# davrempe/contact-human-dynamics

Hardware: NVIDIA H100
Metric: optimised frames/sec (batched phys-optim) (higher is better)
Workload: dtype f64

## Files before the change

### contact-human-dynamics_b200/csrc/chd_api.cu

```cuda
#include <cuda_runtime.h>

#include <cstdio>
#include <cstdlib>
#include <cstring>
#include <vector>

#include "../../include/chd.h"
#include "chd_dev.h"

__global__ void chd_k_stage_begin(ChdDev D);
template <bool GLOBAL>
__global__ void chd_k_eval(ChdDev D);
__global__ void chd_k_init(ChdDev D);
__global__ void chd_k_kkt(ChdDev D);
__global__ void chd_k_kkt_gwin(ChdDev D);
__global__ void chd_k_kcopy(ChdDev D);
__global__ void chd_k_curv(ChdDev D);
__global__ void chd_k_asm(ChdDev D);
__global__ void chd_k_fp64_peak(int mode, int iters, double* sink);
__global__ void chd_k_hess_base(ChdDev D);
__global__ void chd_k_hess_dur(ChdDev D);
__global__ void chd_k_hess_zero(ChdDev D);
__global__ void chd_k_hess_fin(ChdDev D, int mode);
__global__ void chd_k_tables(ChdDev D);
// ... 31 lines not shown
struct chd_phys_batch {
  ChdHostBatch hb;
  ChdDev D;
  std::vector<void*> allocs;
  cudaStream_t stream = nullptr, copy_stream = nullptr;
  cudaEvent_t ev_kkt = nullptr, ev_ls = nullptr, ev_copy = nullptr;
  int64_t launches = 0;
  int timing = 0;
  bool host_only = false;
  double kt_ms[KT_N] = {0};
  int64_t kt_n[KT_N] = {0};
  cudaEvent_t ev0 = nullptr, ev1 = nullptr;
  int* d_frames = nullptr;
  double* d_samples = nullptr;
  ChdIterForm iter = {};
  size_t smem_kkt = 0;
  int kcopy_blocks = 1;
  ChdIpm* h_ipm = nullptr;
  double* d_x0 = nullptr;
  int64_t h2d_bytes = 0;
  ChdStageDev* d_stages = nullptr;
  int sched_max_iter = 0;
  bool sched_has_dur = false;
  double *poly_T0 = nullptr, *poly_tend0 = nullptr, *phase_tend0 = nullptr;
  int* ent_col0 = nullptr;
};

namespace {

template <class T>
// ... 38 lines not shown
    b->launches++;
    b->kt_n[id]++;
    if (b->timing) {
      cudaEventRecord(b->ev1, b->stream);
      cudaEventSynchronize(b->ev1);
      float ms = 0;
      cudaEventElapsedTime(&ms, b->ev0, b->ev1);
      b->kt_ms[id] += ms;
    }
  }
};

void launch_eval(chd_phys_batch* b) {
  Timer t(b, KT_EVAL);
  b->iter.eval<<<b->hb.B, CHD_THREADS, b->iter.smem_eval, b->stream>>>(b->D);
}

int set_schedule(chd_phys_batch* b, const int* sched, int nsched, int override_stage, int override_max_iter) {
  ChdStageDev tab[6];
  for (int s = 0; s < 6; ++s) tab[s] = stage_dev(b->hb.stage[s], s);
  if (override_stage >= 0 && override_max_iter > 0) tab[override_stage].max_iter = override_max_iter;
  CHD_CUDA(cudaMemcpyAsync(b->d_stages, tab, sizeof(tab), cudaMemcpyHostToDevice, b->stream));
  b->D.stages = b->d_stages;
  b->D.nsched = nsched;
  for (int i = 0; i < nsched; ++i) b->D.sched[i] = sched[i];
  b->sched_max_iter = 0;
  b->sched_has_dur = false;
  for (int i = 0; i < nsched; ++i) b->sched_max_iter += tab[sched[i]].max_iter + 2, b->sched_has_dur |= sched[i] == CHD_STAGE_3;
  chd_k_sched_reset<<<(b->hb.B + 127) / 128, 128, 0, b->stream>>>(b->D);
  b->launches++;
  return 0;
}

int run_schedule(chd_phys_batch* b) {
  const int B = b->hb.B;
  const int check_every = 8;
  for (int it = 0; it <= b->sched_max_iter; ++it) {
    {
      Timer t(b, KT_INIT);
      chd_k_stage_begin<<<B, CHD_THREADS, 0, b->stream>>>(b->D);
    }
    launch_eval(b);
    {
      Timer t(b, KT_INIT);
      chd_k_init<<<B, CHD_THREADS, 0, b->stream>>>(b->D);
    }
    {
      Timer t(b, KT_INIT);
      chd_k_hess_zero<<<dim3(8, B), 256, 0, b->stream>>>(b->D);
      chd_k_hess_base<<<dim3(16, B), 256, 0, b->stream>>>(b->D);
      chd_k_hess_fin<<<B, 128, 0, b->stream>>>(b->D, 0);
      b->launches += 2;
    }
    CHD_CUDA(cudaStreamWaitEvent(b->stream, b->ev_copy, 0));
    chd_k_asm<<<dim3(8, B), 256, 0, b->stream>>>(b->D);
    b->launches++;
    {
      Timer t(b, KT_KKT);
      if (b->D.win_smem) chd_k_kkt<<<B, CHD_KKT_THREADS, b->smem_kkt, b->stream>>>(b->D);
      else chd_k_kkt_gwin<<<B, CHD_KKT_THREADS, b->smem_kkt, b->stream>>>(b->D);
    }
    CHD_CUDA(cudaEventRecord(b->ev_kkt, b->stream));
    CHD_CUDA(cudaStreamWaitEvent(b->copy_stream, b->ev_kkt, 0));
    chd_k_kcopy<<<dim3(b->kcopy_blocks, B), 256, 0, b->copy_stream>>>(b->D);
    b->launches++;
    {
      Timer t(b, KT_LS);
      b->iter.linesearch<<<B, CHD_THREADS, b->iter.smem_ls, b->stream>>>(b->D);
    }
    CHD_CUDA(cudaEventRecord(b->ev_ls, b->stream));
    CHD_CUDA(cudaStreamWaitEvent(b->copy_stream, b->ev_ls, 0));
    if (b->sched_has_dur) {
      chd_k_hess_dur<<<dim3(8, B), CHD_THREADS, 0, b->copy_stream>>>(b->D);
      chd_k_hess_fin<<<B, 128, 0, b->copy_stream>>>(b->D, 1);
      b->launches += 2;
    }
    chd_k_curv<<<dim3(8, B), 256, 0, b->copy_stream>>>(b->D);
    b->launches++;
    CHD_CUDA(cudaEventRecord(b->ev_copy, b->copy_stream));
    {
      Timer t(b, KT_SAMPLE);
      chd_k_snapshot<<<B, 128, 0, b->stream>>>(b->D, b->d_frames);
    }
    if ((it % check_every) == check_every - 1) {
      CHD_CUDA(cudaMemcpyAsync(b->h_ipm, b->D.ipm, B * sizeof(ChdIpm), cudaMemcpyDeviceToHost, b->stream));
      CHD_CUDA(cudaStreamSynchronize(b->stream));
      bool any = false;
      for (int i = 0; i < B; ++i) any |= (b->h_ipm[i].phase != CHD_PH_FINISHED);
      if (!any) break;
    }
  }
  CHD_CUDA(cudaMemcpyAsync(b->h_ipm, b->D.ipm, B * sizeof(ChdIpm), cudaMemcpyDeviceToHost, b->stream));
  CHD_CUDA(cudaStreamSynchronize(b->stream));
  CHD_CUDA(cudaStreamSynchronize(b->copy_stream));
  CHD_CUDA(cudaGetLastError());
  return 0;
}

}

extern "C" {

const char* chd_version(void) { return "libchd 0.1 (sm_90a)"; }

// ... 75 lines not shown
  CHD_CUDA(cudaStreamCreateWithFlags(&b->copy_stream, cudaStreamNonBlocking));
  CHD_CUDA(cudaEventCreateWithFlags(&b->ev_kkt, cudaEventDisableTiming));
  CHD_CUDA(cudaEventCreateWithFlags(&b->ev_copy, cudaEventDisableTiming));
  CHD_CUDA(cudaEventCreateWithFlags(&b->ev_ls, cudaEventDisableTiming));
  CHD_CUDA(cudaEventCreate(&b->ev0));
  CHD_CUDA(cudaEventCreate(&b->ev1));
#define UP(field) if ((rc = dev_upload(b, hb.field, &D.field))) return rc;
#define UPM(field, T) if ((rc = dev_upload(b, hb.field, (const T**)&D.field))) return rc;
  UP(seq) UPM(poly_T, double) UPM(poly_tend, double) UP(node_const) UP(par) UP(t_dyn) UP(t_rom) UP(t_data) UP(row_lo) UP(row_hi) UP(node_var)
  UP(itab) UP(ent_ptr) UPM(ent_col, int) UP(ent_row) UP(col_ptr) UP(col_ent) UP(var_kkt) UP(row_kkt) UP(row_set) UP(sets) UPM(phase_tend, double)
  UP(dur0) UP(poly_ph)
  if ((rc = dev_upload(b, hb.poly_T, (const double**)&b->poly_T0))) return rc;
  if ((rc = dev_upload(b, hb.poly_tend, (const double**)&b->poly_tend0))) return rc;
  if ((rc = dev_upload(b, hb.phase_tend, (const double**)&b->phase_tend0))) return rc;
  if ((rc = dev_upload(b, hb.ent_col, (const int**)&b->ent_col0))) return rc;
  if ((rc = dev_upload(b, hb.poly_T, (const double**)&D.poly_Tt))) return rc;
  if ((rc = dev_upload(b, hb.poly_tend, (const double**)&D.poly_tendt))) return rc;
#undef UPM
#undef UP
  const size_t B = hb.B, nm = B * hb.n_max, mm = B * hb.m_max;
#define AL(field, cnt) if ((rc = dev_alloc(b, (cnt), &D.field))) return rc;
  AL(x, nm) AL(xt, nm) AL(jty, nm) AL(unobs, nm) AL(dx, nm) AL(grad, nm) AL(g, mm) AL(gt, mm) AL(Jv, B * hb.slots_max) AL(rflag, mm)
  AL(sc, mm) AL(dL, mm) AL(dU, mm) AL(s, mm) AL(y, mm) AL(zL, mm) AL(zU, mm) AL(ds, mm) AL(dy, mm) AL(dzL, mm) AL(dzU, mm)
  int dev = 0, sms = 0, smem_max = 0;
  CHD_CUDA(cudaGetDevice(&dev));
  CHD_CUDA(cudaDeviceGetAttribute(&sms, cudaDevAttrMultiProcessorCount, dev));
  CHD_CUDA(cudaDeviceGetAttribute(&smem_max, cudaDevAttrMaxSharedMemoryPerBlockOptin, dev));
  cudaFuncAttributes fa_kkt, fa_gwin;
  CHD_CUDA(cudaFuncGetAttributes(&fa_kkt, chd_k_kkt));
  CHD_CUDA(cudaFuncGetAttributes(&fa_gwin, chd_k_kkt_gwin));
  const ChdKktPlan P = chd_kkt_plan(hb.Na_max, hb.nb_max, hb.w_max, hb.w_fix_max, hb.n_max, fa_kkt.sharedSizeBytes,
                                    fa_gwin.sharedSizeBytes, (size_t)smem_max);
  D.win_smem = P.win_smem, D.nbc_max = P.nbc_max, D.Q = P.Q, D.Qfix = P.Qfix, D.nbt = P.nbt, D.win_tiles = P.win_tiles;
  D.pan_doubles = P.pan_doubles, D.kstride = P.kstride, D.scratch_stride = P.scratch_stride;
  b->smem_kkt = P.smem_bytes;
  b->kcopy_blocks = (int)std::min<size_t>(512, std::max<size_t>(std::max<size_t>(1, 4 * (size_t)sms / B), P.kstride * sizeof(double) / 131072));
  AL(cost, B * 2) AL(Kwork, B * P.kstride) AL(Kbase, B * P.kstride) AL(sol, B * (size_t)(hb.Na_max + hb.nb_max)) AL(ipm, B)
  AL(rhs0, B * (size_t)(hb.Na_max + hb.nb_max)) AL(rhs1, B * (size_t)(hb.Na_max + hb.nb_max))
  if (P.scratch_stride) AL(scratch, B * P.scratch_stride)
#undef AL
  if ((rc = dev_upload(b, hb.x0, (const double**)&b->d_x0))) return rc;
  CHD_CUDA(cudaMemcpyAsync(D.x, b->d_x0, nm * sizeof(double), cudaMemcpyDeviceToDevice, b->stream));
  b->iter = chd_iter_form(hb.n_max, smem_max);
  if (P.status == CHD_KKT_TOO_WIDE_COMPACT || P.status == CHD_KKT_TOO_WIDE_PAIRS) {
    fprintf(stderr, "libchd: band + border too wide for the %s (Q=%d nbt=%d)\n",
            P.status == CHD_KKT_TOO_WIDE_COMPACT ? "compacted update loop" : "pair tables", P.Q, P.nbt);
    return -5;
  }
  if (P.status == CHD_KKT_TOO_LARGE) {
    fprintf(stderr, "libchd: KKT band + border too large for the shared memory of the factorisation (n_max=%d)\n", hb.n_max);
    return -5;
  }
  CHD_CUDA(cudaFuncSetAttribute(b->iter.eval, cudaFuncAttributeMaxDynamicSharedMemorySize, (int)b->iter.smem_eval));
  CHD_CUDA(cudaFuncSetAttribute(P.win_smem ? chd_k_kkt : chd_k_kkt_gwin, cudaFuncAttributeMaxDynamicSharedMemorySize, (int)b->smem_kkt));
  CHD_CUDA(cudaFuncSetAttribute(b->iter.linesearch, cudaFuncAttributeMaxDynamicSharedMemorySize, (int)b->iter.smem_ls));
  const size_t stride = 6 + 7 * (size_t)hb.n_ee_max;
  CHD_CUDA(cudaMallocAsync((void**)&b->d_samples, B * hb.fo_max * stride * sizeof(double), b->stream));
  CHD_CUDA(cudaMallocAsync((void**)&b->d_frames, B * sizeof(int), b->stream));
  b->allocs.push_back(b->d_samples);
  b->allocs.push_back(b->d_frames);
  b->h_ipm = (ChdIpm*)std::malloc(B * sizeof(ChdIpm));
  if (!b->h_ipm) return -3;
  CHD_CUDA(cudaMallocAsync((void**)&b->d_stages, 6 * sizeof(ChdStageDev), b->stream));
  b->allocs.push_back(b->d_stages);
  if ((rc = dev_alloc(b, 3 * B * hb.fo_max * stride, &D.snapshots))) return rc;
  CHD_CUDA(cudaStreamSynchronize(b->stream));
  return 0;
}

void chd_phys_batch_destroy(chd_phys_batch* b) {
// ... 217 lines not shown

int64_t chd_phys_launch_count(const chd_phys_batch* b) { return b ? b->launches : 0; }
int64_t chd_phys_h2d_bytes(const chd_phys_batch* b) { return b ? b->h2d_bytes : 0; }
int chd_phys_reset(chd_phys_batch* b) {
  if (!b || b->host_only) return -1;
  CHD_CUDA(cudaMemcpyAsync(b->D.x, b->d_x0, (size_t)b->hb.B * b->hb.n_max * sizeof(double), cudaMemcpyDeviceToDevice, b->stream));
  const ChdHostBatch& hb = b->hb;
  CHD_CUDA(cudaMemcpyAsync(b->D.poly_T, b->poly_T0, hb.poly_T.size() * sizeof(double), cudaMemcpyDeviceToDevice, b->stream));
  CHD_CUDA(cudaMemcpyAsync(b->D.poly_tend, b->poly_tend0, hb.poly_tend.size() * sizeof(double), cudaMemcpyDeviceToDevice, b->stream));
  CHD_CUDA(cudaMemcpyAsync(b->D.phase_tend, b->phase_tend0, hb.phase_tend.size() * sizeof(double), cudaMemcpyDeviceToDevice, b->stream));
  CHD_CUDA(cudaMemcpyAsync(b->D.ent_col, b->ent_col0, hb.ent_col.size() * sizeof(int), cudaMemcpyDeviceToDevice, b->stream));
  chd_k_clear_dyn<<<(hb.B + 127) / 128, 128, 0, b->stream>>>(b->D);
  b->launches++;
  return 0;
}
int chd_phys_set_timing(chd_phys_batch* b, int enable) {
  if (!b) return -1;
  b->timing = enable;
  return 0;
}
int chd_phys_kernel_times(chd_phys_batch* b, double* ms8, int64_t* launches8, int reset) {
  if (!b) return -1;
  for (int i = 0; i < KT_N; ++i) {
    if (ms8) ms8[i] = b->kt_ms[i];
    if (launches8) launches8[i] = b->kt_n[i];
    if (reset) b->kt_ms[i] = 0, b->kt_n[i] = 0;
  }
  return 0;
}

// ... 2 lines not shown
```

### contact-human-dynamics_b200/csrc/chd_dev.h

```cpp
#pragma once
#include "chd_core.h"
#include "chd_kkt_plan.h"
#include "chd_layout.h"

#define CHD_FILT_MAX 24
#define CHD_THREADS 512
#define CHD_NL_GUARD 1.0
#define CHD_NL_FLOOR 1e-4
#define CHD_UNOBS_EPS 1e-14
#define CHD_DW_UNOBS 1e-4
#define CHD_CURV_MIN 1e-8

#define CHD_ROW_ACTIVE 1
#define CHD_ROW_EQ 2
#define CHD_ROW_HASL 4
#define CHD_ROW_HASU 8
#define CHD_ROW_WARM 16

#define CHD_PH_BEGIN 0
#define CHD_PH_RUN 1
#define CHD_PH_FINISHED 2
struct ChdIpm {
  int status;
  int iter, nfilt, ls_fail, max_iter, n_bounds, m_act, pad0;
// ... 71 lines not shown
#define CHD_KAPPA2 1e-2
#define CHD_KAPPA_SIGMA 1e10
#define CHD_S_MAX 100.0
#define CHD_SCAL_MAX_GRAD 100.0
#define CHD_BOUND_RELAX 1e-8
#define CHD_DELTA_W0 1e-4
#define CHD_DELTA_C 1e-8
#define CHD_DW_POLISH 1.0
#define CHD_DW_MIN 1e-8
#define CHD_AF_N 10
#define CHD_AF_MIN 1e-10
#define CHD_DW_MAX 1e4
#define CHD_DW_INC 4.0
#define CHD_DW_DEC 3.0
#define CHD_MAX_BACKTRACK 25
#define CHD_GAMMA_THETA 1e-5
#define CHD_GAMMA_PHI 1e-5
#define CHD_S_PHI 2.3
#define CHD_S_THETA 1.1
#define CHD_ETA_PHI 1e-8
#define CHD_INF 1e19

#if defined(__CUDACC__) || defined(CHD_HOST_EMU)
struct ChdGaps { double L, U; };
__device__ __forceinline__ ChdGaps chd_row_gaps(int f, double s, const double& dL, const double& dU) {
  return {(f & CHD_ROW_HASL) ? s - dL : 1.0, (f & CHD_ROW_HASU) ? dU - s : 1.0};
}
struct ChdSigma {
  double L, U;
  __device__ __forceinline__ double sum() const { return L + U; }
// ... 31 lines not shown
```

### contact-human-dynamics_b200/csrc/chd_eval.cuh

```cuda
#pragma once
#include "chd_dev.h"

struct ChdCtx {
  const ChdSeq* h;
  const double* x;
  const double *poly_T, *poly_tend, *node_const, *par, *t_dyn, *t_rom, *t_data, *dur0;
  const int *node_var, *itab, *ent_ptr, *poly_ph;
  int* ent_col;
  const ChdSet* sets;
  int Pmax, F_max, Ph_max;
  int dyn;
  int opt_dur;
};

__device__ __forceinline__ void chd_make_ctx(const ChdDev& D, int b, const double* x, ChdCtx& c) {
  c.h = D.seq + b;
  c.x = x;
  c.poly_T = D.poly_T + (size_t)b * D.S * D.Pmax;
  c.poly_tend = D.poly_tend + (size_t)b * D.S * D.Pmax;
  c.poly_ph = D.poly_ph + (size_t)b * D.S * D.Pmax;
  c.dur0 = D.dur0 + (size_t)b * D.n_ee_max * D.Ph_max;
  c.ent_col = D.ent_col + (size_t)b * D.slots_max;
  c.Ph_max = D.Ph_max;
  c.dyn = 0;
// ... 570 lines not shown
  for (int w = threadIdx.x; w < 3 * n_ee; w += blockDim.x) {
    const int ee = w % n_ee, kind = w / n_ee;
    const int P = h->n_phases[ee];
    double sum = 0.0, tot = 0.0;
    for (int k = 0; k < P - 1; ++k) sum += x[h->dur_xoff[ee] + k];
    for (int k = 0; k < P; ++k) tot += c.dur0[(size_t)ee * c.Ph_max + k];
    const double last = tot - sum;
    if (kind == 2) {
      if (phase_tend) {
        double t = 0.0;
        for (int k = 0; k < P; ++k) t += k < P - 1 ? x[h->dur_xoff[ee] + k] : last, phase_tend[(size_t)ee * c.Ph_max + k] = t;
      }
      continue;
    }
    const int s = kind == 0 ? chd_sp_motion(ee) : chd_sp_force(n_ee, ee);
    double t = 0.0;
    for (int j = 0; j < h->sp_npoly[s]; ++j) {
      const int info = c.poly_ph[(size_t)s * c.Pmax + j];
      const int ph = info & 4095, npol = info >> 20;
      const double Tj = (ph < P - 1 ? x[h->dur_xoff[ee] + ph] : last) / npol;
      t += Tj;
      polyT[(size_t)s * c.Pmax + j] = Tj;
      polyTend[(size_t)s * c.Pmax + j] = t;
    }
  }
}

__device__ __forceinline__ int chd_set_work(const ChdSet& st, int n_ee, bool jac) {
  return st.type == CHD_SET_DYN ? st.nitems * (jac ? 2 + n_ee : 1) : st.nitems;
}

template <bool JAC>
__device__ void chd_eval_all(const ChdCtx& c, const ChdStageDev& sg, double* g, double* Jv, double* grad, double* cost_out,
                             double* red) {
  const ChdSeq* h = c.h;
  const int n_ee = h->n_ee;
  for (int si = 0; si < h->nsets; ++si) {
    const ChdSet st = c.sets[si];
// ... 43 lines not shown
```

### contact-human-dynamics_b200/csrc/chd_kernels.cu

```cuda
#include <cuda_runtime.h>

#include "chd_block.cuh"
#include "chd_eval.cuh"

__global__ void chd_k_stage_begin(ChdDev D) {
  const int b = blockIdx.x;
  if (D.ipm[b].phase != CHD_PH_BEGIN) return;
  const ChdStageDev sg = D.stages[D.ipm[b].stage];
  const int max_iter = sg.max_iter;
  const ChdSeq* h = D.seq + b;
  if (sg.opt_dur && h->n_dur == 0) {
    __syncthreads();
    if (threadIdx.x == 0) {
      D.ipm[b].iter = 0;
      chd_stage_advance(D, D.ipm[b], -3, sg.snap_after);
    }
    return;
  }
  const bool warm = sg.opt_dur && D.ipm[b].last_p1 == CHD_STAGE_22 + 1;
  int* rf = D.rflag + (size_t)b * D.m_max;
  const double* lo = D.row_lo + (size_t)b * D.m_max;
  const double* hi = D.row_hi + (size_t)b * D.m_max;
  const int* rset = D.row_set + (size_t)b * D.m_max;
  for (int r = threadIdx.x; r < D.m_max; r += blockDim.x) {
// ... 130 lines not shown
    D.zL[ro + r] = hl ? (warm ? mu0 / (s - dL) : 1.0) : 0.0;
    D.zU[ro + r] = hu ? (warm ? mu0 / (dU - s) : 1.0) : 0.0;
    nb_l += (hl ? 1 : 0) + (hu ? 1 : 0);
  }
  const double nbnd = chd_block_sum((double)nb_l, red);
  int act = 0;
  for (int r = threadIdx.x; r < h->m; r += blockDim.x) act += (D.rflag[ro + r] & CHD_ROW_ACTIVE) ? 1 : 0;
  const double nact = chd_block_sum((double)act, red);
  if (threadIdx.x == 0) {
    D.ipm[b].sf = sf;
    D.ipm[b].n_bounds = (int)nbnd;
    D.ipm[b].m_act = (int)nact;
  }
}

template <bool GLOBAL>
__global__ void __launch_bounds__(CHD_THREADS) chd_k_linesearch(ChdDev D) {
  extern __shared__ double sm[];
  __shared__ int s_ok, s_ftype, s_trust;
  __shared__ double s_cost;
  const int b = blockIdx.x;
  ChdIpm& I = D.ipm[b];
  if (I.phase != CHD_PH_RUN || !I.step_ready) return;
  const ChdStageDev sg = D.stages[I.stage];
  const ChdSeq* h = D.seq + b;
  const int n = h->n, m = h->m, tid = threadIdx.x, nt = blockDim.x;
  const size_t ro = (size_t)b * D.m_max, vo = (size_t)b * D.n_max;
  const int* rf = D.rflag + ro;
  double* xt = GLOBAL ? D.xt + vo : sm;
  double* red = GLOBAL ? sm : sm + D.n_max;
  const double* x = D.x + vo;
  const double* dx = D.dx + vo;
  double* gt = D.gt + ro;
  const double mu = I.mu, sf = I.sf, theta = I.theta0, phi0 = I.phi0, dphi = I.dphi, a_pr = I.a_pr, a_du = I.a_du;
  if (a_pr == 0.0 && dphi == 0.0) {
    if (tid == 0) I.iter += 1, I.step_ready = 0;
    return;
  }
  ChdCtx c;
  chd_make_ctx(D, b, xt, c);
  c.dyn = I.dyn;
  c.opt_dur = sg.opt_dur;
  if (sg.opt_dur) {
    c.poly_T = D.poly_Tt + (size_t)b * D.S * D.Pmax;
    c.poly_tend = D.poly_tendt + (size_t)b * D.S * D.Pmax;
    const size_t cnt = (size_t)D.S * D.Pmax;
    for (size_t i = tid; i < cnt; i += nt) {
      D.poly_Tt[(size_t)b * cnt + i] = D.poly_T[(size_t)b * cnt + i];
      D.poly_tendt[(size_t)b * cnt + i] = D.poly_tend[(size_t)b * cnt + i];
    }
    __syncthreads();
  }
  const double theta_ref = I.theta_ref;
  double alpha = a_pr;
  int ls = 0;
  bool accepted = false, ftype = false;
  for (ls = 0; ls < CHD_MAX_BACKTRACK; ++ls) {
    for (int i = tid; i < n; i += nt) xt[i] = x[i] + alpha * dx[i];
    __syncthreads();
    if (sg.opt_dur) {
      if (tid == 0) s_trust = 0;
      __syncthreads();
      if (tid < h->n_ee) {
        double t = 0.0, t0 = 0.0;
        int bad = 0;
        for (int k = 0; k < h->n_phases[tid] - 1; ++k) {
          t += xt[h->dur_xoff[tid] + k];
          t0 += c.dur0[(size_t)tid * c.Ph_max + k];
          if (fabs(t - t0) > CHD_TAU_TRUST) bad = 1;
        }
        if (bad) s_trust = 1;
      }
      chd_tables_from_x(c, xt, D.poly_Tt + (size_t)b * D.S * D.Pmax, D.poly_tendt + (size_t)b * D.S * D.Pmax, nullptr);
      __syncthreads();
    }
    chd_eval_all<false>(c, sg, gt, nullptr, nullptr, &s_cost, red);
    double a_th = 0.0, a_bar = 0.0;
    for (int r = tid; r < m; r += nt) {
      const int f = rf[r];
      if (!(f & CHD_ROW_ACTIVE)) continue;
      const bool eq = f & CHD_ROW_EQ;
      const double st = eq ? 0.0 : D.s[ro + r] + alpha * D.ds[ro + r];
      a_th += fabs(chd_row_res(f, D.sc[ro + r] * gt[r], D.dL[ro + r], st));
      if (!eq) chd_row_barrier(f, mu, chd_row_gaps(f, st, D.dL[ro + r], D.dU[ro + r]), a_bar);
    }
    const double theta_t = chd_block_sum(a_th, red);
    const double bar_t = chd_block_sum(a_bar, red);
    if (tid == 0) {
      const double phit = sf * s_cost + bar_t;
      bool ok = isfinite(phit) && isfinite(theta_t) && theta_t <= I.theta_max;
      if (sg.opt_dur && s_trust) ok = false;
      if (sg.opt_dur && ok && theta_t - (1.0 - alpha) * theta > CHD_NL_GUARD * fmax(alpha * theta, CHD_NL_FLOOR * fmax(1.0, theta_ref))) ok = false;
      for (int q = 0; ok && q < I.nfilt; ++q)
        if (theta_t >= I.filt[2 * q] && phit >= I.filt[2 * q + 1]) ok = false;
      bool acc = false, ft = false;
      if (ok) {
        const bool switching = dphi < 0 && alpha * pow(-dphi, CHD_S_PHI) > pow(theta, CHD_S_THETA);
        const bool armijo = phit <= phi0 + CHD_ETA_PHI * alpha * dphi;
        if (theta <= I.theta_min && switching) {
          if (armijo) acc = true, ft = true;
        } else if (theta_t <= (1 - CHD_GAMMA_THETA) * theta || phit <= phi0 - CHD_GAMMA_PHI * theta) {
          acc = true;
          ft = switching && armijo;
        }
      }
      s_ok = acc, s_ftype = ft;
    }
    __syncthreads();
    accepted = s_ok, ftype = s_ftype;
    __syncthreads();
    if (accepted) break;
    alpha *= 0.5;
  }
  if (!accepted) {
    alpha *= 2.0;
    ls = CHD_MAX_BACKTRACK;
  }
  double* xg = D.x + vo;
  for (int i = tid; i < n; i += nt) xg[i] = xt[i];
  if (sg.opt_dur) {
    __syncthreads();
    chd_tables_from_x(c, xt, D.poly_T + (size_t)b * D.S * D.Pmax, D.poly_tend + (size_t)b * D.S * D.Pmax,
                      D.phase_tend + (size_t)b * D.n_ee_max * D.Ph_max);
  }
  for (int r = tid; r < m; r += nt) {
    const int f = rf[r];
    if (!(f & CHD_ROW_ACTIVE)) continue;
    D.y[ro + r] += alpha * D.dy[ro + r];
    if (f & CHD_ROW_EQ) continue;
    const double s = D.s[ro + r] + alpha * D.ds[ro + r];
    D.s[ro + r] = s;
    const ChdGaps gap = chd_row_gaps(f, s, D.dL[ro + r], D.dU[ro + r]);
    if (f & CHD_ROW_HASL) {
      double z = D.zL[ro + r] + a_du * D.dzL[ro + r];
      z = fmin(fmax(z, mu / (CHD_KAPPA_SIGMA * gap.L)), CHD_KAPPA_SIGMA * mu / gap.L);
      D.zL[ro + r] = z;
    }
    if (f & CHD_ROW_HASU) {
      double z = D.zU[ro + r] + a_du * D.dzU[ro + r];
      z = fmin(fmax(z, mu / (CHD_KAPPA_SIGMA * gap.U)), CHD_KAPPA_SIGMA * mu / gap.U);
      D.zU[ro + r] = z;
    }
  }
  if (tid == 0) {
    if (accepted && !ftype && I.nfilt < CHD_FILT_MAX) {
      I.filt[2 * I.nfilt] = (1 - CHD_GAMMA_THETA) * theta;
      I.filt[2 * I.nfilt + 1] = phi0 - CHD_GAMMA_PHI * theta;
      I.nfilt += 1;
    }
    if (!accepted) I.ls_fail += 1;
    if (!I.af_off) {
      const bool at_floor = ls == 0 && I.delta_w <= I.dw_floor * 1.0000001;
      if (I.dw_floor < CHD_DW_MIN) {
        if (ls > 0 || (I.iter - I.af_it >= 30 && I.E0 > 0.5 * I.af_E)) I.dw_floor = CHD_DW_MIN, I.af_off = 1;
        else if (at_floor && ++I.af_cnt >= CHD_AF_N) I.dw_floor = fmax(I.dw_floor * 0.1, CHD_AF_MIN), I.af_cnt = 0;
      } else if (at_floor) {
        if (++I.af_cnt >= CHD_AF_N) I.dw_floor = fmax(I.dw_floor * 0.1, CHD_AF_MIN), I.af_cnt = 0, I.af_E = I.E0, I.af_it = I.iter;
      } else if (ls > 0) {
        I.af_cnt = 0;
      }
    }
    if (ls == 0) I.delta_w = fmax(I.delta_w / CHD_DW_DEC, I.dw_floor);
    else I.delta_w = fmin(I.delta_w * pow(CHD_DW_INC, (double)min(ls, 3)), CHD_DW_MAX);
    I.iter += 1;
    I.step_ready = 0;
  }
}
template __global__ void chd_k_linesearch<false>(ChdDev D);
template __global__ void chd_k_linesearch<true>(ChdDev D);

__device__ void chd_sample_seq(const ChdDev& D, int b, double* out, int* frames_out) {
  const ChdSeq* h = D.seq + b;
  ChdCtx c;
  chd_make_ctx(D, b, D.x + (size_t)b * D.n_max, c);
  const int n_ee = h->n_ee, stride = 6 + 7 * D.n_ee_max;
  double tot = 0.0;
  for (int k = 0; k < h->sp_npoly[0]; ++k) tot += c.poly_T[k];
  const int nf = (int)((tot + 1e-5) / h->dt) + 1;
  if (threadIdx.x == 0 && frames_out) frames_out[b] = nf;
  double t = 0.0;
  int at = 0;
// ... 73 lines not shown
```

### contact-human-dynamics_b200/phys.py

```python
from __future__ import annotations

import ctypes as C
import os
from typing import List, Optional, Sequence

import numpy as np

from .io_formats import PhysProblem

_HERE = os.path.dirname(os.path.abspath(__file__))
_LIB = None

STAGES = {"1.1": 0, "1.2": 1, "2.1": 2, "2.2": 3, "3": 4, "4": 5}
SET_NAMES = {0: "acc", 1: "terrain", 2: "rom", 3: "dyn", 4: "force", 5: "heel", 6: "height", 7: "tottime", 8: "durpos"}


class _Problem(C.Structure):
    _fields_ = [("n_frames", C.c_int32), ("n_ee", C.c_int32), ("dt", C.c_double),
                ("hip_left", C.POINTER(C.c_double)), ("hip_right", C.POINTER(C.c_double)),
                ("max_leg_length", C.c_double), ("max_heel_length", C.c_double), ("heel_dist", C.c_double),
                ("body_mass", C.c_double), ("inertia", C.POINTER(C.c_double)), ("base_lin", C.POINTER(C.c_double)),
                ("base_ang", C.POINTER(C.c_double)), ("ee_pos", C.POINTER(C.c_double)),
                ("floor_normal", C.c_double * 3), ("floor_point", C.c_double * 3),
                ("ee_start_contact", C.POINTER(C.c_int32)), ("ee_n_phases", C.POINTER(C.c_int32)),
# ... 28 lines not shown
    "chd_phys_eval": (_int, [_vp, _i32, _vp, _vp, _vp, _vp]),
    "chd_phys_get_layout": (_int, [_vp] * 8),
    "chd_phys_get_slot_index": (_int, [_vp] * 4),
    "chd_phys_get_ent_col": (_int, [_vp, _vp]),
    "chd_phys_get_duals": (_int, [_vp] * 7),
    "chd_phys_stage_stats": (_int, [_vp, _vp]),
    "chd_phys_solve_stage": (_int, [_vp, _i32, _i32, _vp, _vp, _vp]),
    "chd_phys_solve": (_int, [_vp] * 6),
    "chd_phys_sample": (_int, [_vp, _vp, _vp]),
    "chd_phys_sample_device": (_int, [_vp, _vp, _vp]),
    "chd_phys_launch_count": (_i64, [_vp]),
    "chd_phys_h2d_bytes": (_i64, [_vp]),
    "chd_phys_reset": (_int, [_vp]),
    "chd_phys_kernel_times": (_int, [_vp, _vp, _vp, _int]),
    "chd_phys_set_timing": (_int, [_vp, _int]),
    "chd_contact_create": (_int, [_vp, _vp, _vp, C.c_float, _i32, C.POINTER(_vp)]),
    "chd_contact_destroy": (None, [_vp]),
    "chd_contact_forward": (_int, [_vp, _vp, _i32, _i32, _vp, _vp, _vp, _vp]),
    "chd_contact_forward_device": (_int, [_vp, _vp, _i32, _i32, _vp, _vp, _vp, _vp, _vp]),
    "chd_contact_preprocess": (_int, [_vp, _vp, _vp, _i32, _f64, _f64, _vp, _vp]),
    "chd_contact_score_device": (_int, [_vp, _vp, _i32, _i32, _vp, _vp, C.c_float, _vp, _vp, _vp, _vp]),
    "chd_contact_detect": (_int, [_vp, _vp, _vp, _i32, _f64, _f64, _vp, _vp, C.c_float, _vp, _vp, _vp, _vp, _vp]),
    "chd_contact_launch_count": (_i64, [_vp]),
    "chd_contact_set_precision": (_int, [_vp, _i32]),
    "chd_openpose_load": (_int, [C.POINTER(C.c_char_p), _i32, _i32, _vp, _i32]),
    "chd_kin_solve": (_int, [_vp] * 7 + [_i32] * 3 + [_vp] * 4),
    "chd_kin_work_bytes": (_i64, [_i32]),
    "chd_ik_solve": (_int, [_i32, _vp, _i32, _vp, _vp, _i32, _i32, _vp, _vp, _vp, _i32, _f64, _f64, _i32, _vp, _vp]),
    "chd_ik_work_bytes": (_i64, [_i32] * 3),
    "chd_version": (C.c_char_p, []),
# ... 200 lines not shown
        self._chk(self.L.chd_phys_sample(self.h, _ptr(out), _ptr(frames)))
        return out, frames

    def launch_count(self) -> int:
        return int(self.L.chd_phys_launch_count(self.h))

    def h2d_bytes(self) -> int:
        return int(self.L.chd_phys_h2d_bytes(self.h))

    def reset(self):
        self._chk(self.L.chd_phys_reset(self.h))

    def set_timing(self, on: bool):
        self.L.chd_phys_set_timing(self.h, int(on))

    def kernel_times(self, reset=False):
        ms, cnt = np.zeros(8), np.zeros(8, np.int64)
        self.L.chd_phys_kernel_times(self.h, _ptr(ms), _ptr(cnt), int(reset))
        names = ["eval", "kkt", "linesearch", "init", "sample"]
        return {k: (float(ms[i]), int(cnt[i])) for i, k in enumerate(names)}

    def _chk(self, rc):
        if rc != 0:
            raise RuntimeError("libchd call failed with code %d" % rc)


SOLUTION_FILES = ("sol_out_no_dynamics.txt", "sol_out_dynamics.txt", "sol_out_durations.txt")


def write_outputs(out: dict, i: int, problem: PhysProblem, out_dir: str, n_ee_max: Optional[int] = None) -> None:
# ... 23 lines not shown
```

### include/chd.h

```cpp
#ifndef CHD_H_
#define CHD_H_
#include <stdint.h>

#ifdef __cplusplus
extern "C" {
#endif

typedef struct chd_phys_problem {
  int32_t n_frames;
  int32_t n_ee;
  double dt;
  const double* hip_left;
  const double* hip_right;
  double max_leg_length, max_heel_length, heel_dist, body_mass;
  const double* inertia;
  const double* base_lin;
  const double* base_ang;
  const double* ee_pos;
  double floor_normal[3], floor_point[3];
  const int32_t* ee_start_contact;
  const int32_t* ee_n_phases;
  const double* ee_durations;
} chd_phys_problem;

// ... 37 lines not shown
                         double* stats);

int chd_phys_solve(chd_phys_batch* b, double* samples, int32_t* frames_out, int32_t* success,
                   int32_t* stage_status, int32_t* stage_iters);

int chd_phys_sample(chd_phys_batch* b, double* out, int32_t* frames_out);

int chd_phys_sample_device(chd_phys_batch* b, double* out_device, void* stream);

int64_t chd_phys_launch_count(const chd_phys_batch* b);
int64_t chd_phys_h2d_bytes(const chd_phys_batch* b);
int chd_phys_reset(chd_phys_batch* b);

int chd_phys_kernel_times(chd_phys_batch* b, double* ms8, int64_t* launches8, int reset);
int chd_phys_set_timing(chd_phys_batch* b, int enable);

typedef struct chd_contact_net chd_contact_net;
int chd_contact_create(const float* weights, const float* biases, const float* bn, float bn_eps, int32_t device,
                       chd_contact_net** out);
void chd_contact_destroy(chd_contact_net* net);
int chd_contact_forward(chd_contact_net* net, const double* frames, int32_t V, int32_t Fmax, const int32_t* seq_lens,
                        int64_t* labels, float* logits, float* min_abs_logit);
int chd_contact_forward_device(chd_contact_net* net, const double* frames_dev, int32_t V, int32_t Fmax,
                               const int32_t* seq_lens_dev, int64_t* labels_dev, float* logits_dev, float* min_abs_dev,
                               void* stream);
int chd_contact_preprocess(chd_contact_net* net, const double* raw, const int32_t* seq_offsets, int32_t V, double scale,
                           double norm, double* frames_out, int32_t* seq_lens_out);
int chd_contact_score_device(chd_contact_net* net, const float* logits_dev, int32_t V, int32_t Fmax, const int32_t* truth_dev,
                             const int32_t* truth_offsets_dev, float classify_thresh, double* loss_sum_dev,
                             int64_t* conf_frames_dev, int64_t* conf_merged_dev, void* stream);
// ... 28 lines not shown
```

Baseline: 13610.

## Evaluate line-search backtracking trials in parallel across thread-block clusters

After: 13880 (median of 6 runs). 1.02x the previous value.

```diff
diff --git a/contact-human-dynamics_b200/csrc/chd_api.cu b/contact-human-dynamics_b200/csrc/chd_api.cu
--- a/contact-human-dynamics_b200/csrc/chd_api.cu
+++ b/contact-human-dynamics_b200/csrc/chd_api.cu
@@ -69,6 +69,11 @@
   int* d_frames = nullptr;
   double* d_samples = nullptr;
   ChdIterForm iter = {};
+  int sms = 0;
+  int ls_tmax = 1;
+  int ls_clusters[CHD_LS_TMAX + 1] = {};
+  int ls_pin = 0;
+  int ls_T = 1;
   size_t smem_kkt = 0;
   int kcopy_blocks = 1;
   ChdIpm* h_ipm = nullptr;
@@ -137,6 +142,34 @@
 void launch_eval(chd_phys_batch* b) {
   Timer t(b, KT_EVAL);
   b->iter.eval<<<b->hb.B, CHD_THREADS, b->iter.smem_eval, b->stream>>>(b->D);
+}
+
+cudaLaunchConfig_t ls_config(const chd_phys_batch* b, int T, cudaLaunchAttribute* attr) {
+  cudaLaunchConfig_t cfg = {};
+  cfg.gridDim = dim3(T, b->hb.B);
+  cfg.blockDim = dim3(CHD_THREADS);
+  cfg.dynamicSmemBytes = b->iter.smem_ls;
+  cfg.stream = b->stream;
+  attr->id = cudaLaunchAttributeClusterDimension;
+  attr->val.clusterDim.x = T, attr->val.clusterDim.y = 1, attr->val.clusterDim.z = 1;
+  cfg.attrs = attr;
+  cfg.numAttrs = 1;
+  return cfg;
+}
+
+int chd_ls_trials(const chd_phys_batch* b, int live) {
+  if (b->ls_pin) return b->ls_pin;
+  int T = std::min(std::max(b->sms / std::max(live, 1), 1), b->ls_tmax);
+  while (T > 1 && b->ls_clusters[T] < live) --T;
+  return T;
+}
+
+int launch_linesearch(chd_phys_batch* b) {
+  Timer t(b, KT_LS);
+  cudaLaunchAttribute attr;
+  const cudaLaunchConfig_t cfg = ls_config(b, b->ls_T, &attr);
+  CHD_CUDA(cudaLaunchKernelEx(&cfg, b->iter.linesearch, b->D));
+  return 0;
 }
 
 int set_schedule(chd_phys_batch* b, const int* sched, int nsched, int override_stage, int override_max_iter) {
@@ -158,6 +191,8 @@
 int run_schedule(chd_phys_batch* b) {
   const int B = b->hb.B;
   const int check_every = 8;
+  int rc = 0;
+  b->ls_T = chd_ls_trials(b, B);
   for (int it = 0; it <= b->sched_max_iter; ++it) {
     {
       Timer t(b, KT_INIT);
@@ -187,10 +222,7 @@
     CHD_CUDA(cudaStreamWaitEvent(b->copy_stream, b->ev_kkt, 0));
     chd_k_kcopy<<<dim3(b->kcopy_blocks, B), 256, 0, b->copy_stream>>>(b->D);
     b->launches++;
-    {
-      Timer t(b, KT_LS);
-      b->iter.linesearch<<<B, CHD_THREADS, b->iter.smem_ls, b->stream>>>(b->D);
-    }
+    if ((rc = launch_linesearch(b))) return rc;
     CHD_CUDA(cudaEventRecord(b->ev_ls, b->stream));
     CHD_CUDA(cudaStreamWaitEvent(b->copy_stream, b->ev_ls, 0));
     if (b->sched_has_dur) {
@@ -208,9 +240,10 @@
     if ((it % check_every) == check_every - 1) {
       CHD_CUDA(cudaMemcpyAsync(b->h_ipm, b->D.ipm, B * sizeof(ChdIpm), cudaMemcpyDeviceToHost, b->stream));
       CHD_CUDA(cudaStreamSynchronize(b->stream));
-      bool any = false;
-      for (int i = 0; i < B; ++i) any |= (b->h_ipm[i].phase != CHD_PH_FINISHED);
-      if (!any) break;
+      int live = 0;
+      for (int i = 0; i < B; ++i) live += b->h_ipm[i].phase != CHD_PH_FINISHED;
+      if (!live) break;
+      b->ls_T = chd_ls_trials(b, live);
     }
   }
   CHD_CUDA(cudaMemcpyAsync(b->h_ipm, b->D.ipm, B * sizeof(ChdIpm), cudaMemcpyDeviceToHost, b->stream));
@@ -316,18 +349,28 @@
   if ((rc = dev_upload(b, hb.poly_tend, (const double**)&b->poly_tend0))) return rc;
   if ((rc = dev_upload(b, hb.phase_tend, (const double**)&b->phase_tend0))) return rc;
   if ((rc = dev_upload(b, hb.ent_col, (const int**)&b->ent_col0))) return rc;
-  if ((rc = dev_upload(b, hb.poly_T, (const double**)&D.poly_Tt))) return rc;
-  if ((rc = dev_upload(b, hb.poly_tend, (const double**)&D.poly_tendt))) return rc;
 #undef UPM
 #undef UP
   const size_t B = hb.B, nm = B * hb.n_max, mm = B * hb.m_max;
 #define AL(field, cnt) if ((rc = dev_alloc(b, (cnt), &D.field))) return rc;
-  AL(x, nm) AL(xt, nm) AL(jty, nm) AL(unobs, nm) AL(dx, nm) AL(grad, nm) AL(g, mm) AL(gt, mm) AL(Jv, B * hb.slots_max) AL(rflag, mm)
-  AL(sc, mm) AL(dL, mm) AL(dU, mm) AL(s, mm) AL(y, mm) AL(zL, mm) AL(zU, mm) AL(ds, mm) AL(dy, mm) AL(dzL, mm) AL(dzU, mm)
   int dev = 0, sms = 0, smem_max = 0;
   CHD_CUDA(cudaGetDevice(&dev));
   CHD_CUDA(cudaDeviceGetAttribute(&sms, cudaDevAttrMultiProcessorCount, dev));
   CHD_CUDA(cudaDeviceGetAttribute(&smem_max, cudaDevAttrMaxSharedMemoryPerBlockOptin, dev));
+  b->sms = sms;
+  b->iter = chd_iter_form(hb.n_max, smem_max);
+  CHD_CUDA(cudaFuncSetAttribute(b->iter.linesearch, cudaFuncAttributeMaxDynamicSharedMemorySize, (int)b->iter.smem_ls));
+  for (int T = 1; T <= CHD_LS_TMAX; ++T) {
+    cudaLaunchAttribute attr;
+    const cudaLaunchConfig_t cfg = ls_config(b, T, &attr);
+    CHD_CUDA(cudaOccupancyMaxActiveClusters(&b->ls_clusters[T], (void*)b->iter.linesearch, &cfg));
+    if (b->ls_clusters[T] > 0) b->ls_tmax = T;
+  }
+  const size_t nt = (size_t)b->ls_tmax;
+  AL(poly_Tt, nt * B * hb.S * hb.Pmax) AL(poly_tendt, nt * B * hb.S * hb.Pmax)
+  AL(x, nm) AL(xt, nt * nm) AL(jty, nm) AL(unobs, nm) AL(dx, nm) AL(grad, nm) AL(g, mm) AL(gt, nt * mm) AL(Jv, B * hb.slots_max)
+  AL(rflag, mm) AL(sc, mm) AL(dL, mm) AL(dU, mm) AL(s, mm) AL(y, mm) AL(zL, mm) AL(zU, mm) AL(ds, mm) AL(dy, mm) AL(dzL, mm)
+  AL(dzU, mm)
   cudaFuncAttributes fa_kkt, fa_gwin;
   CHD_CUDA(cudaFuncGetAttributes(&fa_kkt, chd_k_kkt));
   CHD_CUDA(cudaFuncGetAttributes(&fa_gwin, chd_k_kkt_gwin));
@@ -343,7 +386,6 @@
 #undef AL
   if ((rc = dev_upload(b, hb.x0, (const double**)&b->d_x0))) return rc;
   CHD_CUDA(cudaMemcpyAsync(D.x, b->d_x0, nm * sizeof(double), cudaMemcpyDeviceToDevice, b->stream));
-  b->iter = chd_iter_form(hb.n_max, smem_max);
   if (P.status == CHD_KKT_TOO_WIDE_COMPACT || P.status == CHD_KKT_TOO_WIDE_PAIRS) {
     fprintf(stderr, "libchd: band + border too wide for the %s (Q=%d nbt=%d)\n",
             P.status == CHD_KKT_TOO_WIDE_COMPACT ? "compacted update loop" : "pair tables", P.Q, P.nbt);
@@ -355,7 +397,6 @@
   }
   CHD_CUDA(cudaFuncSetAttribute(b->iter.eval, cudaFuncAttributeMaxDynamicSharedMemorySize, (int)b->iter.smem_eval));
   CHD_CUDA(cudaFuncSetAttribute(P.win_smem ? chd_k_kkt : chd_k_kkt_gwin, cudaFuncAttributeMaxDynamicSharedMemorySize, (int)b->smem_kkt));
-  CHD_CUDA(cudaFuncSetAttribute(b->iter.linesearch, cudaFuncAttributeMaxDynamicSharedMemorySize, (int)b->iter.smem_ls));
   const size_t stride = 6 + 7 * (size_t)hb.n_ee_max;
   CHD_CUDA(cudaMallocAsync((void**)&b->d_samples, B * hb.fo_max * stride * sizeof(double), b->stream));
   CHD_CUDA(cudaMallocAsync((void**)&b->d_frames, B * sizeof(int), b->stream));
@@ -603,6 +644,11 @@
   b->launches++;
   return 0;
 }
+int chd_phys_set_ls_trials(chd_phys_batch* b, int32_t trials) {
+  if (!b || b->host_only || trials < 0 || trials > b->ls_tmax) return -1;
+  b->ls_pin = trials;
+  return 0;
+}
 int chd_phys_set_timing(chd_phys_batch* b, int enable) {
   if (!b) return -1;
   b->timing = enable;
diff --git a/contact-human-dynamics_b200/csrc/chd_dev.h b/contact-human-dynamics_b200/csrc/chd_dev.h
--- a/contact-human-dynamics_b200/csrc/chd_dev.h
+++ b/contact-human-dynamics_b200/csrc/chd_dev.h
@@ -109,6 +109,7 @@
 #define CHD_DW_INC 4.0
 #define CHD_DW_DEC 3.0
 #define CHD_MAX_BACKTRACK 25
+#define CHD_LS_TMAX 8
 #define CHD_GAMMA_THETA 1e-5
 #define CHD_GAMMA_PHI 1e-5
 #define CHD_S_PHI 2.3
diff --git a/contact-human-dynamics_b200/csrc/chd_eval.cuh b/contact-human-dynamics_b200/csrc/chd_eval.cuh
--- a/contact-human-dynamics_b200/csrc/chd_eval.cuh
+++ b/contact-human-dynamics_b200/csrc/chd_eval.cuh
@@ -608,14 +608,25 @@
       continue;
     }
     const int s = kind == 0 ? chd_sp_motion(ee) : chd_sp_force(n_ee, ee);
+    const int np = h->sp_npoly[s], xo = h->dur_xoff[ee];
+    const int* pph = c.poly_ph + (size_t)s * c.Pmax;
     double t = 0.0;
-    for (int j = 0; j < h->sp_npoly[s]; ++j) {
-      const int info = c.poly_ph[(size_t)s * c.Pmax + j];
-      const int ph = info & 4095, npol = info >> 20;
-      const double Tj = (ph < P - 1 ? x[h->dur_xoff[ee] + ph] : last) / npol;
-      t += Tj;
-      polyT[(size_t)s * c.Pmax + j] = Tj;
-      polyTend[(size_t)s * c.Pmax + j] = t;
+    for (int j0 = 0; j0 < np; j0 += 8) {
+      double Tj[8];
+#pragma unroll
+      for (int u = 0; u < 8; ++u) {
+        if (j0 + u >= np) break;
+        const int info = pph[j0 + u];
+        const int ph = info & 4095, npol = info >> 20;
+        Tj[u] = (ph < P - 1 ? x[xo + ph] : last) / npol;
+      }
+#pragma unroll
+      for (int u = 0; u < 8; ++u) {
+        if (j0 + u >= np) break;
+        t += Tj[u];
+        polyT[(size_t)s * c.Pmax + j0 + u] = Tj[u];
+        polyTend[(size_t)s * c.Pmax + j0 + u] = t;
+      }
     }
   }
 }
diff --git a/contact-human-dynamics_b200/csrc/chd_kernels.cu b/contact-human-dynamics_b200/csrc/chd_kernels.cu
--- a/contact-human-dynamics_b200/csrc/chd_kernels.cu
+++ b/contact-human-dynamics_b200/csrc/chd_kernels.cu
@@ -1,7 +1,10 @@
+#include <cooperative_groups.h>
 #include <cuda_runtime.h>
 
 #include "chd_block.cuh"
 #include "chd_eval.cuh"
+
+namespace cg = cooperative_groups;
 
 __global__ void chd_k_stage_begin(ChdDev D) {
   const int b = blockIdx.x;
@@ -168,116 +171,141 @@
   }
 }
 
+__device__ __forceinline__ bool chd_ls_accept(const ChdIpm& I, bool opt_dur, double alpha, double theta_t, double phit,
+                                              int trust, bool* ft) {
+  const double theta = I.theta0, phi0 = I.phi0, dphi = I.dphi;
+  bool ok = isfinite(phit) && isfinite(theta_t) && theta_t <= I.theta_max;
+  if (opt_dur && trust) ok = false;
+  if (opt_dur && ok && theta_t - (1.0 - alpha) * theta > CHD_NL_GUARD * fmax(alpha * theta, CHD_NL_FLOOR * fmax(1.0, I.theta_ref))) ok = false;
+  for (int q = 0; ok && q < I.nfilt; ++q)
+    if (theta_t >= I.filt[2 * q] && phit >= I.filt[2 * q + 1]) ok = false;
+  bool acc = false;
+  *ft = false;
+  if (ok) {
+    const bool switching = dphi < 0 && alpha * pow(-dphi, CHD_S_PHI) > pow(theta, CHD_S_THETA);
+    const bool armijo = phit <= phi0 + CHD_ETA_PHI * alpha * dphi;
+    if (theta <= I.theta_min && switching) {
+      if (armijo) acc = true, *ft = true;
+    } else if (theta_t <= (1 - CHD_GAMMA_THETA) * theta || phit <= phi0 - CHD_GAMMA_PHI * theta) {
+      acc = true;
+      *ft = switching && armijo;
+    }
+  }
+  return acc;
+}
+
 template <bool GLOBAL>
 __global__ void __launch_bounds__(CHD_THREADS) chd_k_linesearch(ChdDev D) {
   extern __shared__ double sm[];
-  __shared__ int s_ok, s_ftype, s_trust;
-  __shared__ double s_cost;
-  const int b = blockIdx.x;
+  __shared__ int s_trust, s_acc, s_ftype;
+  __shared__ double s_cost, s_theta, s_phi;
+  cg::cluster_group cl = cg::this_cluster();
+  const int b = blockIdx.y, rank = (int)cl.block_rank(), T = (int)cl.num_blocks();
   ChdIpm& I = D.ipm[b];
   if (I.phase != CHD_PH_RUN || !I.step_ready) return;
   const ChdStageDev sg = D.stages[I.stage];
   const ChdSeq* h = D.seq + b;
   const int n = h->n, m = h->m, tid = threadIdx.x, nt = blockDim.x;
-  const size_t ro = (size_t)b * D.m_max, vo = (size_t)b * D.n_max;
+  const size_t ro = (size_t)b * D.m_max, vo = (size_t)b * D.n_max, slot = (size_t)rank * D.B + b;
   const int* rf = D.rflag + ro;
-  double* xt = GLOBAL ? D.xt + vo : sm;
+  double* xt = GLOBAL ? D.xt + slot * D.n_max : sm;
   double* red = GLOBAL ? sm : sm + D.n_max;
   const double* x = D.x + vo;
   const double* dx = D.dx + vo;
-  double* gt = D.gt + ro;
+  double* gt = D.gt + slot * D.m_max;
   const double mu = I.mu, sf = I.sf, theta = I.theta0, phi0 = I.phi0, dphi = I.dphi, a_pr = I.a_pr, a_du = I.a_du;
   if (a_pr == 0.0 && dphi == 0.0) {
-    if (tid == 0) I.iter += 1, I.step_ready = 0;
+    if (tid == 0 && rank == 0) I.iter += 1, I.step_ready = 0;
     return;
   }
   ChdCtx c;
   chd_make_ctx(D, b, xt, c);
   c.dyn = I.dyn;
   c.opt_dur = sg.opt_dur;
+  const size_t cnt = (size_t)D.S * D.Pmax;
   if (sg.opt_dur) {
-    c.poly_T = D.poly_Tt + (size_t)b * D.S * D.Pmax;
-    c.poly_tend = D.poly_tendt + (size_t)b * D.S * D.Pmax;
-    const size_t cnt = (size_t)D.S * D.Pmax;
+    c.poly_T = D.poly_Tt + slot * cnt;
+    c.poly_tend = D.poly_tendt + slot * cnt;
     for (size_t i = tid; i < cnt; i += nt) {
-      D.poly_Tt[(size_t)b * cnt + i] = D.poly_T[(size_t)b * cnt + i];
-      D.poly_tendt[(size_t)b * cnt + i] = D.poly_tend[(size_t)b * cnt + i];
+      D.poly_Tt[slot * cnt + i] = D.poly_T[(size_t)b * cnt + i];
+      D.poly_tendt[slot * cnt + i] = D.poly_tend[(size_t)b * cnt + i];
     }
     __syncthreads();
   }
-  const double theta_ref = I.theta_ref;
+  double alpha_w = a_pr;
   double alpha = a_pr;
-  int ls = 0;
-  bool accepted = false, ftype = false;
-  for (ls = 0; ls < CHD_MAX_BACKTRACK; ++ls) {
-    for (int i = tid; i < n; i += nt) xt[i] = x[i] + alpha * dx[i];
-    __syncthreads();
+  int k0 = 0, acc = -1;
+  for (;; k0 += T) {
+    alpha = alpha_w;
+    for (int j = 0; j < rank; ++j) alpha *= 0.5;
+    if (k0 + rank < CHD_MAX_BACKTRACK) {
+      for (int i = tid; i < n; i += nt) xt[i] = x[i] + alpha * dx[i];
+      __syncthreads();
+      if (sg.opt_dur) {
+        if (tid == 0) s_trust = 0;
+        __syncthreads();
+        if (tid < h->n_ee) {
+          double t = 0.0, t0 = 0.0;
+          int bad = 0;
+          for (int k = 0; k < h->n_phases[tid] - 1; ++k) {
+            t += xt[h->dur_xoff[tid] + k];
+            t0 += c.dur0[(size_t)tid * c.Ph_max + k];
+            if (fabs(t - t0) > CHD_TAU_TRUST) bad = 1;
+          }
+          if (bad) s_trust = 1;
+        }
+        chd_tables_from_x(c, xt, D.poly_Tt + slot * cnt, D.poly_tendt + slot * cnt, nullptr);
+        __syncthreads();
+      }
+      chd_eval_all<false>(c, sg, gt, nullptr, nullptr, &s_cost, red);
+      double a_th = 0.0, a_bar = 0.0;
+      for (int r = tid; r < m; r += nt) {
+        const int f = rf[r];
+        if (!(f & CHD_ROW_ACTIVE)) continue;
+        const bool eq = f & CHD_ROW_EQ;
+        const double st = eq ? 0.0 : D.s[ro + r] + alpha * D.ds[ro + r];
+        a_th += fabs(chd_row_res(f, D.sc[ro + r] * gt[r], D.dL[ro + r], st));
+        if (!eq) chd_row_barrier(f, mu, chd_row_gaps(f, st, D.dL[ro + r], D.dU[ro + r]), a_bar);
+      }
+      const double theta_t = chd_block_sum(a_th, red);
+      const double bar_t = chd_block_sum(a_bar, red);
+      if (tid == 0) s_theta = theta_t, s_phi = sf * s_cost + bar_t;
+    }
+    cl.sync();
+    if (rank == 0 && tid == 0) {
+      int a = -1;
+      bool ft = false;
+      double al = alpha_w;
+      for (int j = 0; j < T && k0 + j < CHD_MAX_BACKTRACK; ++j, al *= 0.5) {
+        const double theta_t = *cl.map_shared_rank(&s_theta, j), phit = *cl.map_shared_rank(&s_phi, j);
+        const int trust = sg.opt_dur ? *cl.map_shared_rank(&s_trust, j) : 0;
+        if (chd_ls_accept(I, sg.opt_dur, al, theta_t, phit, trust, &ft)) {
+          a = k0 + j;
+          break;
+        }
+      }
+      if (a < 0 && k0 + T >= CHD_MAX_BACKTRACK) a = CHD_MAX_BACKTRACK;
+      s_acc = a, s_ftype = ft;
+    }
+    cl.sync();
+    acc = *cl.map_shared_rank(&s_acc, 0);
+    if (acc >= 0) break;
+    for (int j = 0; j < T; ++j) alpha_w *= 0.5;
+  }
+  const bool accepted = acc < CHD_MAX_BACKTRACK;
+  const int kacc = accepted ? acc : CHD_MAX_BACKTRACK - 1;
+  if (rank == kacc - k0) {
+    double* xg = D.x + vo;
+    for (int i = tid; i < n; i += nt) xg[i] = xt[i];
     if (sg.opt_dur) {
-      if (tid == 0) s_trust = 0;
       __syncthreads();
-      if (tid < h->n_ee) {
-        double t = 0.0, t0 = 0.0;
-        int bad = 0;
-        for (int k = 0; k < h->n_phases[tid] - 1; ++k) {
-          t += xt[h->dur_xoff[tid] + k];
-          t0 += c.dur0[(size_t)tid * c.Ph_max + k];
-          if (fabs(t - t0) > CHD_TAU_TRUST) bad = 1;
-        }
-        if (bad) s_trust = 1;
-      }
-      chd_tables_from_x(c, xt, D.poly_Tt + (size_t)b * D.S * D.Pmax, D.poly_tendt + (size_t)b * D.S * D.Pmax, nullptr);
-      __syncthreads();
-    }
-    chd_eval_all<false>(c, sg, gt, nullptr, nullptr, &s_cost, red);
-    double a_th = 0.0, a_bar = 0.0;
-    for (int r = tid; r < m; r += nt) {
-      const int f = rf[r];
-      if (!(f & CHD_ROW_ACTIVE)) continue;
-      const bool eq = f & CHD_ROW_EQ;
-      const double st = eq ? 0.0 : D.s[ro + r] + alpha * D.ds[ro + r];
-      a_th += fabs(chd_row_res(f, D.sc[ro + r] * gt[r], D.dL[ro + r], st));
-      if (!eq) chd_row_barrier(f, mu, chd_row_gaps(f, st, D.dL[ro + r], D.dU[ro + r]), a_bar);
-    }
-    const double theta_t = chd_block_sum(a_th, red);
-    const double bar_t = chd_block_sum(a_bar, red);
-    if (tid == 0) {
-      const double phit = sf * s_cost + bar_t;
-      bool ok = isfinite(phit) && isfinite(theta_t) && theta_t <= I.theta_max;
-      if (sg.opt_dur && s_trust) ok = false;
-      if (sg.opt_dur && ok && theta_t - (1.0 - alpha) * theta > CHD_NL_GUARD * fmax(alpha * theta, CHD_NL_FLOOR * fmax(1.0, theta_ref))) ok = false;
-      for (int q = 0; ok && q < I.nfilt; ++q)
-        if (theta_t >= I.filt[2 * q] && phit >= I.filt[2 * q + 1]) ok = false;
-      bool acc = false, ft = false;
-      if (ok) {
-        const bool switching = dphi < 0 && alpha * pow(-dphi, CHD_S_PHI) > pow(theta, CHD_S_THETA);
-        const bool armijo = phit <= phi0 + CHD_ETA_PHI * alpha * dphi;
-        if (theta <= I.theta_min && switching) {
-          if (armijo) acc = true, ft = true;
-        } else if (theta_t <= (1 - CHD_GAMMA_THETA) * theta || phit <= phi0 - CHD_GAMMA_PHI * theta) {
-          acc = true;
-          ft = switching && armijo;
-        }
-      }
-      s_ok = acc, s_ftype = ft;
-    }
-    __syncthreads();
-    accepted = s_ok, ftype = s_ftype;
-    __syncthreads();
-    if (accepted) break;
-    alpha *= 0.5;
-  }
-  if (!accepted) {
-    alpha *= 2.0;
-    ls = CHD_MAX_BACKTRACK;
-  }
-  double* xg = D.x + vo;
-  for (int i = tid; i < n; i += nt) xg[i] = xt[i];
-  if (sg.opt_dur) {
-    __syncthreads();
-    chd_tables_from_x(c, xt, D.poly_T + (size_t)b * D.S * D.Pmax, D.poly_tend + (size_t)b * D.S * D.Pmax,
-                      D.phase_tend + (size_t)b * D.n_ee_max * D.Ph_max);
-  }
-  for (int r = tid; r < m; r += nt) {
+      chd_tables_from_x(c, xt, D.poly_T + (size_t)b * cnt, D.poly_tend + (size_t)b * cnt,
+                        D.phase_tend + (size_t)b * D.n_ee_max * D.Ph_max);
+    }
+  }
+  alpha = alpha_w;
+  for (int j = k0; j < kacc; ++j) alpha *= 0.5;
+  for (int r = rank * nt + tid; r < m; r += T * nt) {
     const int f = rf[r];
     if (!(f & CHD_ROW_ACTIVE)) continue;
     D.y[ro + r] += alpha * D.dy[ro + r];
@@ -296,7 +324,9 @@
       D.zU[ro + r] = z;
     }
   }
-  if (tid == 0) {
+  if (rank == 0 && tid == 0) {
+    const int ls = acc;
+    const bool ftype = s_ftype;
     if (accepted && !ftype && I.nfilt < CHD_FILT_MAX) {
       I.filt[2 * I.nfilt] = (1 - CHD_GAMMA_THETA) * theta;
       I.filt[2 * I.nfilt + 1] = phi0 - CHD_GAMMA_PHI * theta;
@@ -319,6 +349,7 @@
     I.iter += 1;
     I.step_ready = 0;
   }
+  cl.sync();
 }
 template __global__ void chd_k_linesearch<false>(ChdDev D);
 template __global__ void chd_k_linesearch<true>(ChdDev D);
diff --git a/contact-human-dynamics_b200/phys.py b/contact-human-dynamics_b200/phys.py
--- a/contact-human-dynamics_b200/phys.py
+++ b/contact-human-dynamics_b200/phys.py
@@ -66,6 +66,7 @@
     "chd_phys_reset": (_int, [_vp]),
     "chd_phys_kernel_times": (_int, [_vp, _vp, _vp, _int]),
     "chd_phys_set_timing": (_int, [_vp, _int]),
+    "chd_phys_set_ls_trials": (_int, [_vp, _i32]),
     "chd_contact_create": (_int, [_vp, _vp, _vp, C.c_float, _i32, C.POINTER(_vp)]),
     "chd_contact_destroy": (None, [_vp]),
     "chd_contact_forward": (_int, [_vp, _vp, _i32, _i32, _vp, _vp, _vp, _vp]),
@@ -296,6 +297,9 @@
     def set_timing(self, on: bool):
         self.L.chd_phys_set_timing(self.h, int(on))
 
+    def set_ls_trials(self, trials: int):
+        self._chk(self.L.chd_phys_set_ls_trials(self.h, int(trials)))
+
     def kernel_times(self, reset=False):
         ms, cnt = np.zeros(8), np.zeros(8, np.int64)
         self.L.chd_phys_kernel_times(self.h, _ptr(ms), _ptr(cnt), int(reset))
diff --git a/include/chd.h b/include/chd.h
--- a/include/chd.h
+++ b/include/chd.h
@@ -75,6 +75,7 @@
 
 int chd_phys_kernel_times(chd_phys_batch* b, double* ms8, int64_t* launches8, int reset);
 int chd_phys_set_timing(chd_phys_batch* b, int enable);
+int chd_phys_set_ls_trials(chd_phys_batch* b, int32_t trials);
 
 typedef struct chd_contact_net chd_contact_net;
 int chd_contact_create(const float* weights, const float* biases, const float* bn, float bn_eps, int32_t device,
```
